# davidkelley/searchlite

Measured on NVIDIA B200. Metric: bm25_top10_queries_per_sec, higher is better.
Workload: dtype f32

## Files before the change

searchlite_b200/csrc/slg_host.h:

```cpp
#pragma once
#include "../../include/searchlite_gpu.h"

#include <algorithm>
#include <chrono>
#include <cmath>
#include <cstdarg>
#include <cstdio>
#include <cstdlib>
#include <cstring>
#include <limits>
#include <memory>
#include <string>
#include <unordered_map>
#include <vector>

#include <cuda_runtime.h>

#include "slg_launch.h"

namespace slg {

std::string &open_error();

cudaStream_t &pool_stream();
// ... 223 lines not shown
  slg_index *ix = nullptr;
  uint32_t Q = 0, k = 0, cap = 0, U = 0, T = 0;
  slg_exec_t exec = SLG_EXEC_BM25;
  bool matcher = false;
  bool want_stats = false;
  uint64_t posting_count = 0;
  slg::DevBuf slab;
  unsigned char *d_pack = nullptr;
  size_t pack_bytes = 0;
  size_t off_ut_term = 0, off_q_term_off = 0, off_qt_uterm = 0, off_qt_weight = 0, off_qt_group = 0, off_qt_flags = 0,
         off_q_order = 0, off_q_must = 0, off_q_not = 0, off_q_should = 0, off_q_min = 0, off_q_filter = 0,
         off_qt_leaf = 0, off_q_leaves = 0, off_q_plan_off = 0, off_plan_nodes = 0, off_cursor_bounds = 0;
  uint32_t *ut_rng = nullptr;
  float *ut_tile_ub = nullptr;
  unsigned char *state = nullptr;
  size_t state_bytes = 0;
  unsigned long long *thr_key = nullptr, *topk_keys = nullptr, *stats = nullptr, *item_counters = nullptr;
  uint32_t *topk_count = nullptr, *lock = nullptr, *work_counter = nullptr, *n_items = nullptr, *cursor_saw = nullptr;
  slg::QTerm *qterms = nullptr;
  slg::QHead *qheads = nullptr;
  uint2 *items = nullptr;
  slg::ColQ *colq = nullptr;
  uint32_t *ucol = nullptr, *col_slot = nullptr;
  float *ut_max = nullptr;
  slg::ScanPair *scan_pairs = nullptr;
  uint32_t *scan_order = nullptr, *scan_item_start = nullptr, *scan_items = nullptr;
  uint32_t scan_items_cap = 0, scan_chunk = 4096;
  uint32_t max_cols = 0;
  uint8_t *done = nullptr;
  size_t done_bytes = 0;
  uint32_t items_cap = 0;
  unsigned char *results = nullptr;
  size_t result_stride = 0;
  bool staged = false;
  uint32_t max_terms = 0;
  bool use_warp = false, can_items = false, canonical = false;
  bool and_scan = false;
  bool big_k = false;
  unsigned long long *pool_keys = nullptr;
  uint32_t *pool_count = nullptr, *pool_lock = nullptr;
  uint32_t pool_cap = 0;
  bool has_cursor = false;
  std::vector<uint8_t> h_has_cursor;
  uint32_t n_cursor_segs = 0;
  bool has_plan = false;
  uint32_t max_leaves = 1;
// ... 25 lines not shown
```

searchlite_b200/csrc/slg_launch.h:

```cpp
#pragma once
#include "slg_scan_kernel.cuh"

namespace slg {

cudaError_t launch_score_tiles(bool matcher, bool prune, bool stats, bool plan, const SegmentDev &sd, const BatchDev &bd, size_t smem,
                               int grid, cudaStream_t st);
cudaError_t launch_score_warp(bool matcher, bool prune, bool stats, bool staged, bool plan, const SegmentDev &sd, const WarpBatchDev &wb,
                              size_t smem, int grid, cudaStream_t st);
cudaError_t launch_score_items(bool prune, const SegmentDev &sd, const WarpBatchDev &wb, const ItemsDev &it, size_t smem, int grid,
                               cudaStream_t st);
cudaError_t launch_score_sparse(const SegmentDev &sd, const WarpBatchDev &wb, const StreamDev &st_dev, size_t smem, int grid, cudaStream_t st);
cudaError_t launch_score_columns(bool prune, bool pools, const SegmentDev &sd, const WarpBatchDev &wb, const StreamDev &st_dev, size_t smem, int grid, cudaStream_t st);
cudaError_t launch_scan(bool prune, bool pools, const SegmentDev &sd, const WarpBatchDev &wb, const ScanDev &sc, int grid, cudaStream_t st);
cudaError_t launch_columns_pruned(bool pools, const SegmentDev &sd, const WarpBatchDev &wb, const StreamDev &st_dev, int grid, cudaStream_t st);
cudaError_t launch_seed_items(const SegmentDev &sd, const WarpBatchDev &wb, const ItemsDev &it, size_t smem, int grid, cudaStream_t st);

}
```

searchlite_b200/csrc/slg_launch_items.cu:

```cuda
#include "slg_launch.h"

namespace slg {
namespace {
template <class K, class... A>
cudaError_t go(K kern, size_t smem, int grid, cudaStream_t st, A... args) {
  cudaError_t e = cudaFuncSetAttribute(kern, cudaFuncAttributeMaxDynamicSharedMemorySize, (int)smem);
  if (e != cudaSuccess) return e;
  kern<<<grid, kThreads, smem, st>>>(args...);
  return cudaGetLastError();
}
template <class K, class... A>
cudaError_t go_n(K kern, int threads, size_t smem, int grid, cudaStream_t st, A... args) {
  cudaError_t e = cudaFuncSetAttribute(kern, cudaFuncAttributeMaxDynamicSharedMemorySize, (int)smem);
  if (e != cudaSuccess) return e;
  kern<<<grid, threads, smem, st>>>(args...);
  return cudaGetLastError();
}
}

cudaError_t launch_score_items(bool prune, const SegmentDev &sd, const WarpBatchDev &wb, const ItemsDev &it, size_t smem, int grid,
                               cudaStream_t st) {
  return prune ? go(slg_score_items_kernel<true>, smem, grid, st, sd, wb, it) : go(slg_score_items_kernel<false>, smem, grid, st, sd, wb, it);
}
cudaError_t launch_score_sparse(const SegmentDev &sd, const WarpBatchDev &wb, const StreamDev &st_dev, size_t smem, int grid, cudaStream_t st) {
  cudaError_t e = cudaFuncSetAttribute(slg_score_sparse_kernel<false>, cudaFuncAttributeMaxDynamicSharedMemorySize, (int)smem);
  if (e != cudaSuccess) return e;
  slg_score_sparse_kernel<false><<<grid, kSparseWarps * 32, smem, st>>>(sd, wb, st_dev);
  return cudaGetLastError();
}
cudaError_t launch_score_columns(bool prune, bool pools, const SegmentDev &sd, const WarpBatchDev &wb, const StreamDev &st_dev, size_t smem, int grid,
                                 cudaStream_t st) {
  if (pools)
    return prune ? go_n(slg_score_columns_kernel<true, true>, kColWarps * 32, smem, grid, st, sd, wb, st_dev)
                 : go_n(slg_score_columns_kernel<false, true>, kColWarps * 32, smem, grid, st, sd, wb, st_dev);
  return prune ? go_n(slg_score_columns_kernel<true, false>, kColWarps * 32, smem, grid, st, sd, wb, st_dev)
               : go_n(slg_score_columns_kernel<false, false>, kColWarps * 32, smem, grid, st, sd, wb, st_dev);
}
cudaError_t launch_columns_pruned(bool pools, const SegmentDev &sd, const WarpBatchDev &wb, const StreamDev &st_dev, int grid, cudaStream_t st) {
  if (pools) slg_columns_pruned_kernel<1><<<grid, 256, 0, st>>>(sd, wb, st_dev);
  else slg_columns_pruned_kernel<0><<<grid, 256, 0, st>>>(sd, wb, st_dev);
  return cudaGetLastError();
}
template <bool PRUNE, bool POOLS>
static void launch_scan_pm(bool must, const SegmentDev &sd, const WarpBatchDev &wb, const ScanDev &sc, int grid, cudaStream_t st) {
  if (must) slg_scan_kernel<PRUNE, POOLS, true><<<grid, kScanWarps * 32, 0, st>>>(sd, wb, sc);
  else slg_scan_kernel<PRUNE, POOLS, false><<<grid, kScanWarps * 32, 0, st>>>(sd, wb, sc);
}
cudaError_t launch_scan(bool prune, bool pools, const SegmentDev &sd, const WarpBatchDev &wb, const ScanDev &sc, int grid, cudaStream_t st) {
  const bool must = sc.must_mode != 0u;
  if (pools) {
    if (prune) launch_scan_pm<true, true>(must, sd, wb, sc, grid, st);
    else launch_scan_pm<false, true>(must, sd, wb, sc, grid, st);
  } else {
    if (prune) launch_scan_pm<true, false>(must, sd, wb, sc, grid, st);
    else launch_scan_pm<false, false>(must, sd, wb, sc, grid, st);
  }
  return cudaGetLastError();
}
cudaError_t launch_seed_items(const SegmentDev &sd, const WarpBatchDev &wb, const ItemsDev &it, size_t smem, int grid, cudaStream_t st) {
  return go(slg_seed_items_kernel<0>, smem, grid, st, sd, wb, it);
}
}
```

searchlite_b200/csrc/slg_scan_kernel.cuh:

```cuda
#pragma once
#include "slg_stream_kernel.cuh"

namespace slg {

constexpr uint32_t kScanChunk = 4096;
constexpr int kScanWarps = 8;
constexpr uint32_t kScanQueue = 512;

struct __align__(16) ScanPair {
  uint64_t base;
  uint32_t df;
  uint32_t qslot_t;
  uint32_t qi;
  float w;
  float others;
  float ne_prefix;
  int32_t filter;
  uint32_t first_item;
  uint32_t pad[2];
};

struct ScanDev {
  const uint32_t *ut_term;
  float *ut_max;
// ... 22 lines not shown
  const uint32_t df = seg.term_df[term];
  const uint32_t quads = (df + 3) >> 2;
  const uint32_t per = (quads + gridDim.y - 1) / gridDim.y;
  const uint32_t q0 = blockIdx.y * per, q1 = min(quads, q0 + per);
  if (q0 >= q1) return;
  const float4 *p = reinterpret_cast<const float4 *>(seg.post_score + seg.term_start[term]);
  uint32_t m = 0u;
  for (uint32_t i = q0 + lane; i < q1; i += 32) {
    const float4 v = __ldg(p + i);
    m = max(m, max(max(__float_as_uint(v.x), __float_as_uint(v.y)), max(__float_as_uint(v.z), __float_as_uint(v.w))));
  }
  m = __reduce_max_sync(0xFFFFFFFFu, m);
  if (lane == 0 && m) atomicMax(reinterpret_cast<uint32_t *>(sc.ut_max) + u, m);
}

static __global__ void slg_term_ub_gather_kernel(SegmentDev seg, ScanDev sc, uint32_t n_uterms) {
  const uint32_t u = blockIdx.x * blockDim.x + threadIdx.x;
  if (u >= n_uterms) return;
  const uint32_t term = sc.ut_term[u];
  sc.ut_max[u] = term < seg.n_terms ? seg.term_ub[term] : 0.0f;
}

constexpr uint32_t kColSlices = 64;
template <int POOLS>
__global__ void __launch_bounds__(256) slg_columns_pruned_kernel(SegmentDev seg, WarpBatchDev wb, StreamDev sd) {
  __shared__ __align__(16) unsigned long long s_cand[8][kWarpCand];
  __shared__ uint32_t s_hist[8][POOLS ? 256 : 1];
  const int lane = threadIdx.x & 31, warp = threadIdx.x >> 5;
  const uint32_t n_colq = *sd.n_colq;
  const uint32_t wid = blockIdx.x * 8 + warp;
  const uint32_t qidx = wid / kColSlices, slice = wid % kColSlices;
  if (qidx >= n_colq) return;
  const ColQ cq = sd.colq[qidx];
  const QTerm *qts = wb.qterms + (uint64_t)cq.qslot * kWarpMaxTerms;
  const uint32_t nt = (uint32_t)cq.nsp + cq.ncol;
  const uint32_t n_blocks = (seg.doc_count + 511u) >> 9;
  const uint32_t per = (n_blocks + kColSlices - 1) / kColSlices;
  const uint32_t b0 = slice * per, b1 = min(n_blocks, b0 + per);
  WarpCand wc;
  wc.begin(s_cand[warp], load_threshold(wb, cq.qi), wb.k, lane, 1u, POOLS ? s_hist[warp] : nullptr);
  auto cut_of = [&]() {
    if (wc.thr == kThrInit) return 0u;
    const float cf = __uint_as_float((uint32_t)(wc.thr >> 32)) * 0.99998f - cq.extra * 1.00002f;
    return cf > 0.0f ? __float_as_uint(cf) : 0u;
  };
  for (uint32_t bb = b0; bb < b1; bb += 32) {
    const uint32_t blk = bb + lane;
    float bound = 0.0f;
    if (blk < b1)
      for (uint32_t i = 0; i < cq.ncol; i++) {
        const QTerm &q = qts[cq.nsp + i];
        bound = __fadd_rn(bound, __fmul_rn(__ldg(seg.col_tmax + (uint64_t)q.term * seg.tmax_stride + blk), q.weight));
      }
    uint32_t open = __ballot_sync(0xFFFFFFFFu, blk < b1 && bound != 0.0f && __float_as_uint(bound) >= cut_of());
    while (open) {
      const uint32_t d0 = (bb + (__ffs(open) - 1)) << 9;
      open &= open - 1;
      float4 v[4];
#pragma unroll
      for (int x = 0; x < 4; x++) v[x] = make_float4(0, 0, 0, 0);
      for (uint32_t i = 0; i < cq.ncol; i++) {
        const QTerm &q = qts[cq.nsp + i];
        const float4 *p = reinterpret_cast<const float4 *>(seg.cols + q.sc_base + d0) + lane;
        const float w = q.weight;
#pragma unroll
        for (int x = 0; x < 4; x++) {
          const float4 c = __ldg(p + x * 32);
          v[x].x = __fadd_rn(v[x].x, __fmul_rn(c.x, w));
          v[x].y = __fadd_rn(v[x].y, __fmul_rn(c.y, w));
          v[x].z = __fadd_rn(v[x].z, __fmul_rn(c.z, w));
          v[x].w = __fadd_rn(v[x].w, __fmul_rn(c.w, w));
        }
      }
      uint32_t cut = cut_of();
      uint32_t todo = 0u;
#pragma unroll
      for (int x = 0; x < 4; x++) {
        const uint32_t bx[4] = {__float_as_uint(v[x].x), __float_as_uint(v[x].y), __float_as_uint(v[x].z), __float_as_uint(v[x].w)};
#pragma unroll
        for (int e = 0; e < 4; e++)
          if (bx[e] >= cut && bx[e] != 0u && d0 + x * 128 + lane * 4 + e < seg.doc_count) todo |= 1u << (x * 4 + e);
      }
      while (__any_sync(0xFFFFFFFFu, todo != 0u)) {
        const uint32_t el = todo ? __ffs(todo) - 1 : 0u;
        const bool had = todo != 0u;
        todo &= todo - 1u;
        uint32_t bits = 0u;
#pragma unroll
        for (int x = 0; x < 4; x++) {
          if (el == (uint32_t)x * 4 + 0) bits = __float_as_uint(v[x].x);
          if (el == (uint32_t)x * 4 + 1) bits = __float_as_uint(v[x].y);
          if (el == (uint32_t)x * 4 + 2) bits = __float_as_uint(v[x].z);
          if (el == (uint32_t)x * 4 + 3) bits = __float_as_uint(v[x].w);
        }
        const uint32_t doc = d0 + (el >> 2) * 128 + lane * 4 + (el & 3u);
        cut = cut_of();
        const bool pass = had && bits >= cut;
        if (!__any_sync(0xFFFFFFFFu, pass)) continue;
        float s = __uint_as_float(bits);
        if (cq.nsp) {
          uint32_t holders = 0u;
          s = verify_doc(seg, wb, qts, nt, pass, doc, holders);
        }
        wc.offer(seg, wb, cq.qi, cq.filter, pass, doc, s);
      }
    }
  }
  wc.merge(wb, cq.qi);
}

static __global__ void __launch_bounds__(128) slg_scan_pairs_kernel(SegmentDev seg, WarpBatchDev wb, ScanDev sc, uint32_t dbg) {
  const uint32_t qslot = blockIdx.x * blockDim.x + threadIdx.x;
  if (qslot >= wb.n_queries) return;
  const QHead h = wb.qheads[qslot];
  float ub[kWarpMaxTerms];
  bool is_col[kWarpMaxTerms];
  for (uint32_t t = 0; t < kWarpMaxTerms; t++) {
    ub[t] = 0.0f;
    is_col[t] = false;
    if (t < h.nt) {
      const QTerm &q = wb.qterms[(uint64_t)qslot * kWarpMaxTerms + t];
      if (q.flags & 1u) ub[t] = __fmul_rn(sc.ut_max[q.uterm], q.weight);
      is_col[t] = (q.flags & 4u) != 0u;
    }
  }
  uint32_t driver = 0xFFFFFFFFu;
  float total_ub = 0.0f;
  if (sc.must_mode) {
    uint32_t best_df = 0xFFFFFFFFu;
    bool possible = h.nt > 0;
    for (uint32_t t = 0; t < h.nt && t < kWarpMaxTerms; t++) {
// ... 358 lines not shown
```

searchlite_b200/csrc/slg_search.cu:

```cuda
#include "slg_host.h"
#include "slg_residency.cuh"

using namespace slg;

namespace {

struct TermSet {
  std::vector<uint32_t> key, val;
  uint32_t mask = 0;
  explicit TermSet(size_t expect) {
    size_t n = 64;
    while (n < expect * 2) n <<= 1;
    key.assign(n, 0xFFFFFFFFu);
    val.assign(n, 0);
    mask = (uint32_t)n - 1;
  }
  uint32_t get(uint32_t term, std::vector<uint32_t> &ut) {
    uint32_t h = (term * 0x9E3779B1u) & mask;
    for (;;) {
      if (key[h] == term) return val[h];
      if (key[h] == 0xFFFFFFFFu) {
        key[h] = term;
        val[h] = (uint32_t)ut.size();
        ut.push_back(term);
        return val[h];
      }
// ... 245 lines not shown
    bt->off_q_leaves = place(n_queries);
    bt->off_q_plan_off = place((size_t)(n_queries + 1) * 4);
    bt->off_plan_nodes = place(plan_nodes.size() * sizeof(PlanNodeDev));
  }
  if (bt->has_cursor) bt->off_cursor_bounds = place(bounds.size() * 8);
  bt->pack_bytes = pos;

  size_t dpos = 0;
  auto carve = [&](size_t bytes) {
    size_t o = dpos;
    dpos = align_up(dpos + std::max<size_t>(bytes, 16), 256);
    return o;
  };
  const size_t o_pack = carve(bt->pack_bytes);
  const size_t o_rng = carve((size_t)std::max(bt->U, 1u) * (max_tiles + 1) * 4);
  const size_t o_ub = (exec != SLG_EXEC_BM25 || bt->can_items) ? carve((size_t)std::max(bt->U, 1u) * max_tiles * 4) : 0;
  uint32_t kp = 1;
  while (kp < k) kp <<= 1;
  bt->pool_cap = bt->big_k ? 2 * kp : 0;
  const size_t state_words = (size_t)n_queries * 2 + 64 + 2 + (bt->big_k ? (size_t)n_queries * 4 : 0);
  const size_t o_thr = carve((size_t)n_queries * 8 + state_words * 4);
  const size_t o_topk = carve((size_t)n_queries * k * 8);
  const size_t o_pools = bt->big_k ? carve((size_t)n_queries * 2 * bt->pool_cap * 8) : 0;
  const size_t o_stats = carve((size_t)n_queries * 5 * 8 + 64);
  const size_t o_saw = bt->has_cursor ? carve((size_t)n_queries * 4) : 0;
  const size_t o_qterms = bt->use_warp ? carve((size_t)n_queries * kWarpMaxTerms * sizeof(QTerm)) : 0;
  const size_t o_qheads = bt->use_warp ? carve((size_t)n_queries * sizeof(QHead)) : 0;
  const bool want_items = bt->can_items && exec != SLG_EXEC_BM25;
  bt->items_cap = want_items ? max_groups * n_queries : 0;
  bt->done_bytes = want_items ? (size_t)max_groups * n_queries : 0;
  const size_t o_items = want_items ? carve((size_t)bt->items_cap * sizeof(uint2)) : 0;
  const bool want_stream = bt->can_items && ix->stream_kernels;
  for (auto &s : ix->segs) bt->max_cols = std::max(bt->max_cols, s->n_cols);
  {
    uint32_t max_docs = 0;
    for (auto &sg : ix->segs) max_docs = std::max(max_docs, sg->doc_count);
    bt->scan_chunk = ix->scan_chunk ? ix->scan_chunk : (max_docs >= 4000000u ? 4096u : max_docs >= 2000000u ? 2048u : 1024u);
  }
  if (bt->can_items) {
    for (auto &sg : ix->segs) {
      uint64_t n = 0;
      for (size_t i = 0; i < qt_u.size(); i++) {
        const uint32_t term = ut[qt_u[i]];
        if (term >= sg->n_terms || !qt_f[i]) continue;
        if (!bt->and_scan && !sg->h_term_col.empty() && sg->h_term_col[term] >= 0) continue;
        n += (sg->h_df[term] + bt->scan_chunk - 1) / bt->scan_chunk;
      }
      bt->scan_items_cap = (uint32_t)std::max<uint64_t>(bt->scan_items_cap, std::min<uint64_t>(n, 0xFFFFFFF0ull));
    }
  }
  const bool want_scan = bt->can_items;
  const size_t o_utmax = want_scan ? carve((size_t)std::max(bt->U, 1u) * 4) : 0;
  const size_t o_pairs = want_scan ? carve((size_t)n_queries * kWarpMaxTerms * sizeof(ScanPair)) : 0;
  const size_t o_order = want_scan ? carve((size_t)n_queries * kWarpMaxTerms * 4) : 0;
  const size_t o_istart = want_scan ? carve(((size_t)n_queries * kWarpMaxTerms + 1) * 4) : 0;
  const size_t o_sitems = want_scan ? carve((size_t)std::max(bt->scan_items_cap, 1u) * 4) : 0;
  const size_t o_colq = want_stream ? carve((size_t)n_queries * sizeof(ColQ)) : 0;
  const size_t o_ucol = want_stream ? carve((size_t)(bt->max_cols + 1) * 4) : 0;
  const size_t o_colslot = want_stream ? carve((size_t)(bt->max_cols + 1) * 4) : 0;
  const size_t o_done = want_items ? carve(bt->done_bytes) : 0;
  bt->result_stride = align_up((size_t)n_queries * k * sizeof(HitDev) + (size_t)n_queries * 4 + (size_t)n_queries * k * 4, 256);
  const size_t o_results = carve(bt->result_stride * (S + (S > 1 ? 1 : 0)));
  SLG_CUDA(ix, bt->slab.alloc(dpos));
  unsigned char *base = bt->slab.as<unsigned char>();
  bt->d_pack = base + o_pack;
  bt->ut_rng = reinterpret_cast<uint32_t *>(base + o_rng);
  bt->ut_tile_ub = (exec != SLG_EXEC_BM25 || bt->can_items) ? reinterpret_cast<float *>(base + o_ub) : nullptr;
  bt->thr_key = reinterpret_cast<unsigned long long *>(base + o_thr);
  bt->state = base + o_thr + (size_t)n_queries * 8;
  bt->state_bytes = state_words * 4;
  bt->topk_count = reinterpret_cast<uint32_t *>(bt->state);
  bt->lock = bt->topk_count + n_queries;
  bt->work_counter = bt->lock + n_queries;
  bt->n_items = bt->work_counter + 64;
  bt->pool_count = bt->big_k ? bt->n_items + 2 : nullptr;
  bt->pool_lock = bt->big_k ? bt->pool_count + (size_t)n_queries * 2 : nullptr;
  bt->pool_keys = bt->big_k ? reinterpret_cast<unsigned long long *>(base + o_pools) : nullptr;
  bt->topk_keys = reinterpret_cast<unsigned long long *>(base + o_topk);
  bt->stats = reinterpret_cast<unsigned long long *>(base + o_stats);
  bt->item_counters = bt->stats + (size_t)n_queries * 5;
  bt->cursor_saw = bt->has_cursor ? reinterpret_cast<uint32_t *>(base + o_saw) : nullptr;
  bt->qterms = bt->use_warp ? reinterpret_cast<QTerm *>(base + o_qterms) : nullptr;
  bt->qheads = bt->use_warp ? reinterpret_cast<QHead *>(base + o_qheads) : nullptr;
  bt->items = want_items ? reinterpret_cast<uint2 *>(base + o_items) : nullptr;
  bt->done = want_items ? base + o_done : nullptr;
  bt->ut_max = want_scan ? reinterpret_cast<float *>(base + o_utmax) : nullptr;
  bt->scan_pairs = want_scan ? reinterpret_cast<ScanPair *>(base + o_pairs) : nullptr;
  bt->scan_order = want_scan ? reinterpret_cast<uint32_t *>(base + o_order) : nullptr;
  bt->scan_item_start = want_scan ? reinterpret_cast<uint32_t *>(base + o_istart) : nullptr;
  bt->scan_items = want_scan ? reinterpret_cast<uint32_t *>(base + o_sitems) : nullptr;
  bt->colq = want_stream ? reinterpret_cast<ColQ *>(base + o_colq) : nullptr;
  bt->ucol = want_stream ? reinterpret_cast<uint32_t *>(base + o_ucol) : nullptr;
  bt->col_slot = want_stream ? reinterpret_cast<uint32_t *>(base + o_colslot) : nullptr;
  bt->results = base + o_results;

  bt->pinned_result_off = align_up(bt->pack_bytes, 256);
  bt->pinned_bytes = bt->pinned_result_off + bt->result_stride + (size_t)n_queries * 40 + 64;
  if (!ix->pinned_busy && ix->pinned && ix->pinned_bytes >= bt->pinned_bytes) {
    bt->pinned = ix->pinned;
    bt->pinned_from_index = true;
    ix->pinned_busy = true;
  } else {
    SLG_CUDA(ix, cudaMallocHost(&bt->pinned, bt->pinned_bytes));
  }
  unsigned char *hp = static_cast<unsigned char *>(bt->pinned);
  auto put = [&](size_t off, const void *src, size_t bytes) {
    if (bytes) std::memcpy(hp + off, src, bytes);
  };
  put(bt->off_ut_term, ut.data(), (size_t)bt->U * 4);
  put(bt->off_q_term_off, q_off.data(), (size_t)(n_queries + 1) * 4);
  put(bt->off_qt_uterm, qt_u.data(), (size_t)bt->T * 4);
  put(bt->off_qt_weight, qt_w.data(), (size_t)bt->T * 4);
  put(bt->off_qt_group, qt_g.data(), bt->T);
  put(bt->off_qt_flags, qt_f.data(), bt->T);
  put(bt->off_q_order, order.data(), (size_t)n_queries * 4);
  put(bt->off_q_must, q_must.data(), n_queries);
  put(bt->off_q_not, q_not.data(), n_queries);
  put(bt->off_q_should, q_should.data(), n_queries);
  put(bt->off_q_min, q_min.data(), n_queries);
  put(bt->off_q_filter, q_filter.data(), (size_t)n_queries * 4);
// ... 20 lines not shown
  const bool prune = bt->exec != SLG_EXEC_BM25;
  const uint32_t Q = bt->Q, k = bt->k;
  const bool run_items = bt->can_items && !bt->want_stats && !(bt->big_k && (!ix->scan_kernels || (ix->strict_accumulate && bt->exec == SLG_EXEC_BM25)));
  const bool run_scan = run_items && ix->scan_kernels && bt->colq != nullptr && !(ix->strict_accumulate && !prune);
  if (bt->and_scan && !run_scan && run_items)
    return fail(ix, SLG_ERR_UNSUPPORTED, "an AND batch prepared for the posting scan cannot run on the sub-tile kernels (strict_accumulate)");
  const bool two_step = !(do_seeds && do_sweep);
  if (two_step && (ix->segs.size() != 1 || !run_items || (!prune && !run_scan)))
    return fail(ix, SLG_ERR_UNSUPPORTED, "the two-step run (first part, threshold exchange, rest) needs one segment per handle and the posting scan or the pruned items kernel");
  unsigned char *dp = bt->d_pack;
  size_t smem = 0;
  const bool run_scan_pre = bt->can_items && !bt->want_stats && ix->scan_kernels && bt->colq != nullptr && !(ix->strict_accumulate && !prune);
  const bool warp_path = bt->use_warp && !(bt->big_k && !run_scan_pre);
  if (!warp_path) {
    int32_t rc = bt->has_plan ? select_smem(ix, bt->plan_docs, bt->cap, bt->matcher, &smem, bt->max_leaves)
                              : select_smem(ix, ix->tile_docs, bt->cap, bt->matcher, &smem);
    if (rc) return rc;
  }
  uint32_t per_sm = (uint32_t)std::max<size_t>(1, (ix->smem_optin + 1024) / (smem + 1024));
  per_sm = std::min(per_sm, 8u);
  if (ix->ctas_per_sm) per_sm = std::min(per_sm, ix->ctas_per_sm);
  if (do_seeds) {
    SLG_CUDA(ix, cudaEventRecord(ix->ev[0], st));
    SLG_CUDA(ix, cudaMemsetAsync(bt->stats, 0, (size_t)Q * 40 + 64, st));
    if (bt->has_cursor) {
      if (bt->n_cursor_segs != ix->segs.size()) return fail(ix, SLG_ERR_INVALID, "a segment was loaded after the batch with cursors was prepared");
      SLG_CUDA(ix, cudaMemsetAsync(bt->cursor_saw, 0, (size_t)Q * 4, st));
    }
  }
  uint32_t si = 0;
  for (auto &sp : ix->segs) {
    Segment *s = sp.get();
    BatchDev bd{};
    bd.ut_term = reinterpret_cast<const uint32_t *>(dp + bt->off_ut_term);
    bd.ut_rng = bt->ut_rng;
    bd.ut_tile_ub = bt->ut_tile_ub;
    bd.q_term_off = reinterpret_cast<const uint32_t *>(dp + bt->off_q_term_off);
    bd.qt_uterm = reinterpret_cast<const uint32_t *>(dp + bt->off_qt_uterm);
    bd.qt_weight = reinterpret_cast<const float *>(dp + bt->off_qt_weight);
    bd.qt_group = dp + bt->off_qt_group;
    bd.qt_flags = dp + bt->off_qt_flags;
    bd.q_order = reinterpret_cast<const uint32_t *>(dp + bt->off_q_order);
    bd.q_must = dp + bt->off_q_must;
    bd.q_not = dp + bt->off_q_not;
    bd.q_should = dp + bt->off_q_should;
    bd.q_min_should = dp + bt->off_q_min;
    bd.q_filter = reinterpret_cast<const int32_t *>(dp + bt->off_q_filter);
// ... 127 lines not shown
      sc.ut_max = bt->ut_max;
      sc.pairs = bt->scan_pairs;
      sc.order = bt->scan_order;
      sc.n_pairs = bt->work_counter + 5;
      sc.n_items = bt->work_counter + 6;
      sc.item_start = bt->scan_item_start;
      sc.items = bt->scan_items;
      sc.items_cap = bt->scan_items_cap;
      sc.chunk = bt->scan_chunk;
      sc.must_mode = bt->and_scan ? 1u : 0u;
      sc.counter = bt->work_counter + 7;
      sc.counters = bt->item_counters;
      StreamDev sdv{};
      sdv.colq = bt->colq;
      sdv.n_colq = bt->work_counter + 3;
      sdv.ucol = bt->ucol;
      sdv.n_ucol = bt->work_counter + 4;
      sdv.col_slot = bt->col_slot;
      sdv.sparse_counter = bt->work_counter + 1;
      sdv.col_counter = bt->work_counter + 2;
      sdv.stage_cap = ix->stage_cap;
      sdv.strict = 0;
      sdv.counters = bt->item_counters;
      if (do_seeds) {
        if (prune && s->dev.term_ub) {
          slg_term_ub_gather_kernel<<<(bt->U + 255) / 256, 256, 0, st>>>(s->dev, sc, bt->U);
        } else {
          SLG_CUDA(ix, cudaMemsetAsync(bt->ut_max, 0, (size_t)bt->U * 4, st));
          slg_term_max_kernel<<<dim3((bt->U + 7) / 8, kMaxSlices), 256, 0, st>>>(s->dev, sc, bt->U);
        }
        slg_scan_pairs_kernel<<<(Q + 127) / 128, 128, 0, st>>>(s->dev, wb, sc, ix->dbg);
        slg_scan_order_kernel<<<1, 1024, 0, st>>>(wb, sc);
        if (bt->scan_items_cap) slg_scan_items_kernel<<<(bt->scan_items_cap + 255) / 256, 256, 0, st>>>(sc);
        for (int i = 0; i < 4; i++) count_launch(ix);
        SLG_CUDA(ix, cudaGetLastError());
        SLG_CUDA(ix, cudaEventRecord(ix->ev[2], st));
      }
      sc.two_rounds = (ix->dbg & 8u) ? 1u : 0u;
      sc.part_lo = do_seeds ? 0u : ix->scan_first_part;
      sc.part_hi = do_sweep ? 256u : ix->scan_first_part;
      SLG_CUDA(ix, launch_scan(prune, wb.pool_keys != nullptr, s->dev, wb, sc, ix->n_sm * 4, st));
      count_launch(ix);
      if (do_sweep && s->n_cols && !(ix->dbg & 4u) && !bt->and_scan) {
        slg_colgroups_kernel<<<1, 1024, 0, st>>>(s->dev, wb, sdv, s->n_cols, prune ? bt->ut_max : nullptr);
        count_launch(ix);
        SLG_CUDA(ix, cudaGetLastError());
        sdv.n_smax = std::min(s->n_cols, kColMaxSlots);
        const size_t fixed = column_smem(0, sdv.n_smax);
        const size_t reserve = 2048 + (size_t)kColWarps * 256 * 4;
        const size_t budget = ix->smem_optin > fixed + reserve ? ix->smem_optin - fixed - reserve : 0;
        sdv.col_resident = (uint32_t)std::min<size_t>(s->n_cols, budget / (2 * kColBlock * 4));
        const size_t csmem = column_smem(sdv.col_resident, sdv.n_smax);
        const uint32_t n_cblocks = (s->doc_count + kColBlock - 1) / kColBlock;
        if (prune) {
          (void)csmem;
          (void)n_cblocks;
          SLG_CUDA(ix, launch_columns_pruned(wb.pool_keys != nullptr, s->dev, wb, sdv, (int)((Q * kColSlices + 7) / 8), st));
        } else {
          SLG_CUDA(ix, launch_score_columns(false, wb.pool_keys != nullptr, s->dev, wb, sdv, csmem, (int)std::min<uint32_t>((uint32_t)ix->n_sm, n_cblocks), st));
        }
        count_launch(ix);
      }
      if (do_sweep) ix->ctr.score_launches++;
    }
    if (do_sweep) {
      if (score && run_scan) {
      } else if (score && run_stream) {
        StreamDev sdv{};
        sdv.colq = bt->colq;
        sdv.n_colq = bt->work_counter + 3;
        sdv.ucol = bt->ucol;
        sdv.n_ucol = bt->work_counter + 4;
        sdv.col_slot = bt->col_slot;
        sdv.sparse_counter = bt->work_counter + 1;
        sdv.col_counter = bt->work_counter + 2;
        sdv.stage_cap = ix->stage_cap;
        sdv.strict = ix->strict_accumulate;
        sdv.counters = bt->item_counters;
        const size_t ssmem = (size_t)kSparseWarps * sparse_smem_per_warp(wb.sub_docs, sdv.stage_cap);
        if (ssmem + 1024 > ix->smem_optin) return fail(ix, SLG_ERR_UNSUPPORTED, "sub_docs %u with stage_cap %u needs %zu B shared memory", wb.sub_docs, sdv.stage_cap, ssmem);
// ... 177 lines not shown
}

int32_t slg_batch_device_results(slg_batch_t *bt, void **dev_hits, void **dev_counts) {
  if (!bt || !dev_hits || !dev_counts) return SLG_ERR_INVALID;
  unsigned char *r = result_block(bt);
  *dev_hits = r;
  *dev_counts = r + (size_t)bt->Q * bt->k * sizeof(HitDev);
  return SLG_OK;
}

int32_t slg_batch_packed_results(slg_batch_t *bt, void **dev_block, uint64_t *n_bytes) {
  if (!bt || !dev_block || !n_bytes) return SLG_ERR_INVALID;
  *dev_block = result_block(bt);
  *n_bytes = (uint64_t)bt->Q * bt->k * sizeof(HitDev) + (uint64_t)bt->Q * 4 + (bt->reranked ? (uint64_t)bt->Q * bt->k * 4 : 0);
  return SLG_OK;
}

int32_t slg_batch_fetch(slg_batch_t *bt, slg_hit_t *out_hits, uint32_t *out_counts, slg_stats_t *out_stats) {
  if (!bt || !out_hits || !out_counts) return SLG_ERR_INVALID;
  slg_index *ix = bt->ix;
  SLG_CUDA(ix, cudaSetDevice(ix->device));
  cudaStream_t st = ix->stream;
  static_assert(sizeof(slg_hit_t) == sizeof(HitDev), "hit layout");
  const size_t hb = (size_t)bt->Q * bt->k * sizeof(slg_hit_t), cb = (size_t)bt->Q * 4, sb = (size_t)bt->Q * 40 + 64;
  unsigned char *pin = static_cast<unsigned char *>(bt->pinned) + bt->pinned_result_off;
  SLG_CUDA(ix, cudaMemcpyAsync(pin, result_block(bt), hb + cb, cudaMemcpyDeviceToHost, st));
  SLG_CUDA(ix, cudaMemcpyAsync(pin + bt->result_stride, bt->stats, sb, cudaMemcpyDeviceToHost, st));
  SLG_CUDA(ix, cudaStreamSynchronize(st));
  ix->ctr.last_d2h_bytes = hb + cb + sb;
  std::memcpy(out_hits, pin, hb);
  std::memcpy(out_counts, pin + hb, cb);
  const unsigned long long *sv = reinterpret_cast<const unsigned long long *>(pin + bt->result_stride);
  const unsigned long long *ic = sv + (size_t)bt->Q * 5;
  ix->ctr.last_postings_scattered = ic[0];
  ix->ctr.last_subtiles_skipped = ic[1];
  ix->ctr.last_column_blocks_streamed = ic[2];
  ix->ctr.last_items = ic[3];
  ix->ctr.last_postings_verified = ic[4];
  ix->ctr.last_items_dropped = ic[5];
  if (getenv("SLG_SCAN_TRACE"))
    fprintf(stderr, "[slg scan] verified %llu, sparse look-ups answered by a presence bitmap %llu, by lower_bound_interp %llu\n", ic[4], ic[6], ic[7]);
  if (out_stats) {
    for (uint32_t q = 0; q < bt->Q; q++) {
      out_stats[q].scored_docs = sv[q * 4 + 0];
      out_stats[q].postings_advanced = sv[q * 4 + 1];
      out_stats[q].blocks_skipped = sv[q * 4 + 2];
      out_stats[q].candidates_examined = sv[q * 4 + 3];
      out_stats[q].total_matches = sv[(size_t)bt->Q * 4 + q];
    }
  }
  return SLG_OK;
}

int32_t slg_batch_copy_results_device(slg_batch_t *bt, void *dst_hits, void *dst_counts) {
  if (!bt || !dst_hits || !dst_counts) return SLG_ERR_INVALID;
  slg_index *ix = bt->ix;
  SLG_CUDA(ix, cudaSetDevice(ix->device));
  void *dh, *dc;
  slg_batch_device_results(bt, &dh, &dc);
  SLG_CUDA(ix, cudaMemcpyAsync(dst_hits, dh, (size_t)bt->Q * bt->k * sizeof(HitDev), cudaMemcpyDeviceToDevice, ix->stream));
  SLG_CUDA(ix, cudaMemcpyAsync(dst_counts, dc, (size_t)bt->Q * 4, cudaMemcpyDeviceToDevice, ix->stream));
  return SLG_OK;
}

// ... 115 lines not shown
```

searchlite_b200/csrc/slg_stream_kernel.cuh:

```cuda
#pragma once
#include "slg_async.cuh"
#include "slg_items_kernel.cuh"
#include "slg_residency.cuh"

namespace slg {

constexpr uint32_t kColBlock = 256;
constexpr int kSparseWarps = 4;
constexpr int kColWarps = 16;
constexpr uint32_t kColMaxSlots = 4096;

struct __align__(16) ColQ {
  uint32_t qslot, qi;
  int32_t filter;
  uint8_t nsp, ncol, unit_w, off;
  uint16_t slot[8];
  float extra;
  uint32_t pad[3];
};

struct StreamDev {
  ColQ *colq;
  uint32_t *n_colq;
  uint32_t *ucol;
  uint32_t *n_ucol;
  uint32_t *col_slot;
  uint32_t *sparse_counter, *col_counter;
  uint32_t stage_cap;
  uint32_t col_resident;
  uint32_t n_smax;
  uint32_t strict;
  unsigned long long *counters;
};

__device__ __forceinline__ bool colq_prune(const WarpBatchDev &wb, const float *ut_max, uint32_t qslot, uint32_t qi, uint32_t nt, float &extra) {
  const unsigned long long thr = load_threshold(wb, qi);
  float ub[kWarpMaxTerms];
  bool col[kWarpMaxTerms];
  for (uint32_t t = 0; t < kWarpMaxTerms; t++) {
    ub[t] = 0.0f;
    col[t] = false;
    if (t < nt) {
      const QTerm &q = wb.qterms[(uint64_t)qslot * kWarpMaxTerms + t];
      if (q.flags & 1u) ub[t] = __fmul_rn(ut_max[q.uterm], q.weight);
      col[t] = (q.flags & 5u) == 5u;
    }
  }
  extra = 0.0f;
  bool any_essential_col = false;
  for (uint32_t t = 0; t < nt; t++) {
    float pre = 0.0f;
    for (uint32_t u = 0; u < nt; u++)
      if (ub[u] < ub[t] || (ub[u] == ub[t] && u >= t)) pre += ub[u];
    const bool ne = thr != kThrInit && pre * 1.00002f < __uint_as_float((uint32_t)(thr >> 32));
    if (col[t]) any_essential_col = any_essential_col || !ne;
// ... 45 lines not shown
          sd.col_slot[c] = 0xFFFFFFFFu;
        }
      }
      __syncthreads();
      if (tid == nthr - 1) s_carry += s_scan[tid];
      __syncthreads();
    }
    if (tid == 0) *sd.n_ucol = s_carry;
  }
  __syncthreads();
  for (uint32_t slot = tid; slot < wb.n_queries; slot += nthr) {
    const QHead h = wb.qheads[slot];
    ColQ r;
    r.qslot = slot;
    r.qi = h.qi;
    r.filter = h.filter;
    r.nsp = 0;
    r.ncol = 0;
    r.unit_w = 1;
    r.off = 0;
    r.extra = 0.0f;
    r.pad[0] = r.pad[1] = r.pad[2] = 0;
    for (int i = 0; i < 8; i++) r.slot[i] = 0;
    for (uint32_t t = 0; t < h.nt; t++) {
      const QTerm &q = wb.qterms[(uint64_t)slot * kWarpMaxTerms + t];
      if (!(q.flags & 1u)) continue;
      if (q.flags & 4u) {
        r.slot[r.ncol++] = (uint16_t)sd.col_slot[q.term];
        if (q.weight != 1.0f) r.unit_w = 0;
      } else {
        r.nsp++;
      }
    }
    if (r.ncol && ut_max) {
      if (!colq_prune(wb, ut_max, slot, h.qi, h.nt, r.extra)) continue;
      bool all_in = true;
      for (uint32_t i = 0; i < r.ncol; i++) all_in = all_in && r.slot[i] != 0xFFFFu;
      if (!all_in) r.off = 1;
    }
    if (r.ncol && !r.off) sd.colq[atomicAdd(sd.n_colq, 1u)] = r;
  }
}

__device__ __forceinline__ uint32_t warp_dedupe64(unsigned long long *a, int lane) {
  const unsigned long long x0 = a[lane], x1 = a[lane + 32];
  const unsigned long long p0 = lane ? a[lane - 1] : ~0ull, p1 = a[lane + 31];
  const bool k0 = x0 != 0ull && x0 != p0, k1 = x1 != 0ull && x1 != p1;
  const uint32_t b0 = __ballot_sync(0xFFFFFFFFu, k0), b1 = __ballot_sync(0xFFFFFFFFu, k1);
  const uint32_t lt = (1u << lane) - 1u, n0 = __popc(b0), n = n0 + __popc(b1);
  __syncwarp();
  if (k0) a[__popc(b0 & lt)] = x0;
  if (k1) a[n0 + __popc(b1 & lt)] = x1;
  __syncwarp();
  for (uint32_t z = n + lane; z < kWarpCand; z += 32) a[z] = 0ull;
  __syncwarp();
  return n;
}

struct WarpCand {
  unsigned long long *cand;
  unsigned long long thr;
  uint32_t cnt;
  uint32_t k;
// ... 78 lines not shown
    if (k1 <= thr) k1 = 0ull;
    const uint32_t b0 = __ballot_sync(0xFFFFFFFFu, k0 != 0ull), b1 = __ballot_sync(0xFFFFFFFFu, k1 != 0ull);
    const uint32_t n_new = __popc(b0) + __popc(b1);
    cnt = 0;
    __syncwarp();
    if (n_new == 0) return;
    const uint32_t slot = qi * 2u + pool;
    unsigned long long *pk = wb.pool_keys + (uint64_t)slot * wb.pool_cap;
    if (lane == 0) {
      while (atomicCAS(wb.pool_lock + slot, 0u, 1u) != 0u) __nanosleep(64);
      __threadfence();
    }
    __syncwarp();
    uint32_t n = ld_cg_u32(wb.pool_count + slot);
    if (n + n_new > wb.pool_cap) n = compact_pool(wb, qi, pk, n);
    const uint32_t lt = (1u << lane) - 1u;
    const uint32_t w0 = __ballot_sync(0xFFFFFFFFu, k0 > thr), w1 = __ballot_sync(0xFFFFFFFFu, k1 > thr);
    if (k0 > thr) st_cg_u64(pk + n + __popc(w0 & lt), k0);
    if (k1 > thr) st_cg_u64(pk + n + __popc(w0) + __popc(w1 & lt), k1);
    __threadfence();
    __syncwarp();
    if (lane == 0) {
      st_cg_u32(wb.pool_count + slot, n + __popc(w0) + __popc(w1));
      __threadfence();
      atomicExch(wb.pool_lock + slot, 0u);
    }
    __syncwarp();
  }
  __device__ __forceinline__ void push(bool pass, unsigned long long key) {
    const uint32_t bal = __ballot_sync(0xFFFFFFFFu, pass);
    if (!bal) return;
    if (pass) cand[cnt + __popc(bal & ((1u << lane) - 1u))] = key;
    cnt += __popc(bal);
    __syncwarp();
    if (cnt > 32 && hist) {
      return;
    }
    if (cnt > 32) {
      for (uint32_t z = cnt + lane; z < kWarpCand; z += 32) cand[z] = 0ull;
      __syncwarp();
      warp_sort64_desc(cand, lane);
      cnt = min(warp_dedupe64(cand, lane), k);
      if (cnt == k) thr = max(thr, cand[k - 1]);
      __syncwarp();
    }
  }
// ... 775 lines not shown
```

Before: 593,100.

## Seed column-pruned scoring with best-bound blocks per query to raise thresholds early

```diff
diff --git a/searchlite_b200/csrc/slg_host.h b/searchlite_b200/csrc/slg_host.h
--- a/searchlite_b200/csrc/slg_host.h
+++ b/searchlite_b200/csrc/slg_host.h
@@ -269,6 +269,7 @@
   uint2 *items = nullptr;
   slg::ColQ *colq = nullptr;
   uint32_t *ucol = nullptr, *col_slot = nullptr;
+  uint32_t *col_seeded = nullptr;
   float *ut_max = nullptr;
   slg::ScanPair *scan_pairs = nullptr;
   uint32_t *scan_order = nullptr, *scan_item_start = nullptr, *scan_items = nullptr;
diff --git a/searchlite_b200/csrc/slg_launch.h b/searchlite_b200/csrc/slg_launch.h
--- a/searchlite_b200/csrc/slg_launch.h
+++ b/searchlite_b200/csrc/slg_launch.h
@@ -12,7 +12,7 @@
 cudaError_t launch_score_sparse(const SegmentDev &sd, const WarpBatchDev &wb, const StreamDev &st_dev, size_t smem, int grid, cudaStream_t st);
 cudaError_t launch_score_columns(bool prune, bool pools, const SegmentDev &sd, const WarpBatchDev &wb, const StreamDev &st_dev, size_t smem, int grid, cudaStream_t st);
 cudaError_t launch_scan(bool prune, bool pools, const SegmentDev &sd, const WarpBatchDev &wb, const ScanDev &sc, int grid, cudaStream_t st);
-cudaError_t launch_columns_pruned(bool pools, const SegmentDev &sd, const WarpBatchDev &wb, const StreamDev &st_dev, int grid, cudaStream_t st);
+cudaError_t launch_columns_pruned(bool pools, const SegmentDev &sd, const WarpBatchDev &wb, const StreamDev &st_dev, uint32_t n_queries, cudaStream_t st);
 cudaError_t launch_seed_items(const SegmentDev &sd, const WarpBatchDev &wb, const ItemsDev &it, size_t smem, int grid, cudaStream_t st);
 
 }
diff --git a/searchlite_b200/csrc/slg_launch_items.cu b/searchlite_b200/csrc/slg_launch_items.cu
--- a/searchlite_b200/csrc/slg_launch_items.cu
+++ b/searchlite_b200/csrc/slg_launch_items.cu
@@ -36,9 +36,15 @@
   return prune ? go_n(slg_score_columns_kernel<true, false>, kColWarps * 32, smem, grid, st, sd, wb, st_dev)
                : go_n(slg_score_columns_kernel<false, false>, kColWarps * 32, smem, grid, st, sd, wb, st_dev);
 }
-cudaError_t launch_columns_pruned(bool pools, const SegmentDev &sd, const WarpBatchDev &wb, const StreamDev &st_dev, int grid, cudaStream_t st) {
-  if (pools) slg_columns_pruned_kernel<1><<<grid, 256, 0, st>>>(sd, wb, st_dev);
-  else slg_columns_pruned_kernel<0><<<grid, 256, 0, st>>>(sd, wb, st_dev);
+cudaError_t launch_columns_pruned(bool pools, const SegmentDev &sd, const WarpBatchDev &wb, const StreamDev &st_dev, uint32_t n_queries, cudaStream_t st) {
+  const int grid = (int)(((uint64_t)n_queries * kColSlices + 7) / 8);
+  if (pools) {
+    slg_columns_seed_kernel<1><<<n_queries, kColSeeds, 0, st>>>(sd, wb, st_dev);
+    slg_columns_pruned_kernel<1><<<grid, 256, 0, st>>>(sd, wb, st_dev);
+  } else {
+    slg_columns_seed_kernel<0><<<n_queries, kColSeeds, 0, st>>>(sd, wb, st_dev);
+    slg_columns_pruned_kernel<0><<<grid, 256, 0, st>>>(sd, wb, st_dev);
+  }
   return cudaGetLastError();
 }
 template <bool PRUNE, bool POOLS>
diff --git a/searchlite_b200/csrc/slg_scan_kernel.cuh b/searchlite_b200/csrc/slg_scan_kernel.cuh
--- a/searchlite_b200/csrc/slg_scan_kernel.cuh
+++ b/searchlite_b200/csrc/slg_scan_kernel.cuh
@@ -68,6 +68,126 @@
 }
 
 constexpr uint32_t kColSlices = 64;
+#ifndef SLG_COL_SEED_WARPS
+#define SLG_COL_SEED_WARPS 8
+#endif
+constexpr uint32_t kColSeedWarps = SLG_COL_SEED_WARPS;
+constexpr uint32_t kColSeeds = kColSeedWarps * 32;
+constexpr int kSeedBatch = 8;
+
+__device__ __forceinline__ uint32_t col_cut(unsigned long long thr, float extra) {
+  if (thr == kThrInit) return 0u;
+  const float cf = __uint_as_float((uint32_t)(thr >> 32)) * 0.99998f - extra * 1.00002f;
+  return cf > 0.0f ? __float_as_uint(cf) : 0u;
+}
+
+__device__ __forceinline__ void col_score_block(const SegmentDev &seg, const WarpBatchDev &wb, const ColQ &cq, const QTerm *qts, uint32_t d0,
+                                                WarpCand &wc, int lane) {
+  const uint32_t nt = (uint32_t)cq.nsp + cq.ncol;
+  float4 v[4];
+#pragma unroll
+  for (int x = 0; x < 4; x++) v[x] = make_float4(0, 0, 0, 0);
+  for (uint32_t i = 0; i < cq.ncol; i++) {
+    const QTerm &q = qts[cq.nsp + i];
+    const float4 *p = reinterpret_cast<const float4 *>(seg.cols + q.sc_base + d0) + lane;
+    const float w = q.weight;
+#pragma unroll
+    for (int x = 0; x < 4; x++) {
+      const float4 c = __ldg(p + x * 32);
+      v[x].x = __fadd_rn(v[x].x, __fmul_rn(c.x, w));
+      v[x].y = __fadd_rn(v[x].y, __fmul_rn(c.y, w));
+      v[x].z = __fadd_rn(v[x].z, __fmul_rn(c.z, w));
+      v[x].w = __fadd_rn(v[x].w, __fmul_rn(c.w, w));
+    }
+  }
+  uint32_t cut = col_cut(wc.thr, cq.extra);
+  uint32_t todo = 0u;
+#pragma unroll
+  for (int x = 0; x < 4; x++) {
+    const uint32_t bx[4] = {__float_as_uint(v[x].x), __float_as_uint(v[x].y), __float_as_uint(v[x].z), __float_as_uint(v[x].w)};
+#pragma unroll
+    for (int e = 0; e < 4; e++)
+      if (bx[e] >= cut && bx[e] != 0u && d0 + x * 128 + lane * 4 + e < seg.doc_count) todo |= 1u << (x * 4 + e);
+  }
+  while (__any_sync(0xFFFFFFFFu, todo != 0u)) {
+    const uint32_t el = todo ? __ffs(todo) - 1 : 0u;
+    const bool had = todo != 0u;
+    todo &= todo - 1u;
+    uint32_t bits = 0u;
+#pragma unroll
+    for (int x = 0; x < 4; x++) {
+      if (el == (uint32_t)x * 4 + 0) bits = __float_as_uint(v[x].x);
+      if (el == (uint32_t)x * 4 + 1) bits = __float_as_uint(v[x].y);
+      if (el == (uint32_t)x * 4 + 2) bits = __float_as_uint(v[x].z);
+      if (el == (uint32_t)x * 4 + 3) bits = __float_as_uint(v[x].w);
+    }
+    const uint32_t doc = d0 + (el >> 2) * 128 + lane * 4 + (el & 3u);
+    cut = col_cut(wc.thr, cq.extra);
+    const bool pass = had && bits >= cut;
+    if (!__any_sync(0xFFFFFFFFu, pass)) continue;
+    float s = __uint_as_float(bits);
+    if (cq.nsp) {
+      uint32_t holders = 0u;
+      s = verify_doc(seg, wb, qts, nt, pass, doc, holders);
+    }
+    wc.offer(seg, wb, cq.qi, cq.filter, pass, doc, s);
+  }
+}
+
+template <int POOLS>
+__global__ void __launch_bounds__(kColSeedWarps * 32, 1) slg_columns_seed_kernel(SegmentDev seg, WarpBatchDev wb, StreamDev sd) {
+  __shared__ __align__(16) unsigned long long s_cand[kColSeedWarps][kWarpCand];
+  __shared__ uint32_t s_hist[kColSeedWarps][POOLS ? 256 : 1];
+  const int lane = threadIdx.x & 31, warp = threadIdx.x >> 5;
+  const uint32_t qidx = blockIdx.x, g = threadIdx.x;
+  if (qidx >= *sd.n_colq) return;
+  const ColQ cq = sd.colq[qidx];
+  const QTerm *qts = wb.qterms + (uint64_t)cq.qslot * kWarpMaxTerms;
+  const uint32_t n_blocks = (seg.doc_count + 511u) >> 9;
+  float best = 0.0f;
+  uint32_t best_blk = 0xFFFFFFFFu;
+  for (uint32_t b0 = g; b0 < n_blocks; b0 += kColSeeds * kSeedBatch) {
+    float bnd[kSeedBatch];
+#pragma unroll
+    for (int j = 0; j < kSeedBatch; j++) bnd[j] = 0.0f;
+    for (uint32_t i = 0; i < cq.ncol; i++) {
+      const QTerm &q = qts[cq.nsp + i];
+      const float *tm = seg.col_tmax + (uint64_t)q.term * seg.tmax_stride;
+      const float w = q.weight;
+#pragma unroll
+      for (int j = 0; j < kSeedBatch; j++) {
+        const uint32_t blk = b0 + j * kColSeeds;
+        if (blk < n_blocks) bnd[j] = __fadd_rn(bnd[j], __fmul_rn(__ldg(tm + blk), w));
+      }
+    }
+#pragma unroll
+    for (int j = 0; j < kSeedBatch; j++)
+      if (bnd[j] > best) {
+        best = bnd[j];
+        best_blk = b0 + j * kColSeeds;
+      }
+  }
+  sd.seeded[(uint64_t)qidx * kColSeeds + g] = best_blk;
+  WarpCand wc;
+  wc.begin(s_cand[warp], load_threshold(wb, cq.qi), wb.k, lane, 1u, POOLS ? s_hist[warp] : nullptr);
+  bool left = best_blk != 0xFFFFFFFFu;
+  uint32_t n_open = 0;
+  for (;;) {
+    wc.thr = max(wc.thr, load_threshold(wb, cq.qi));
+    const uint32_t bits = left ? __float_as_uint(best) : 0u;
+    const uint32_t top = __reduce_max_sync(0xFFFFFFFFu, bits);
+    if (top == 0u || top < col_cut(wc.thr, cq.extra)) break;
+    const uint32_t owner = __ffs(__ballot_sync(0xFFFFFFFFu, left && bits == top)) - 1;
+    if (lane == (int)owner) left = false;
+    const uint32_t blk = __shfl_sync(0xFFFFFFFFu, best_blk, owner);
+    n_open++;
+    col_score_block(seg, wb, cq, qts, blk << 9, wc, lane);
+  }
+  if (POOLS) wc.publish_pool(wb, cq.qi);
+  else wc.merge(wb, cq.qi);
+  if (sd.counters && lane == 0 && n_open) atomicAdd(sd.counters + 1, (unsigned long long)n_open);
+}
+
 template <int POOLS>
 __global__ void __launch_bounds__(256) slg_columns_pruned_kernel(SegmentDev seg, WarpBatchDev wb, StreamDev sd) {
   __shared__ __align__(16) unsigned long long s_cand[8][kWarpCand];
@@ -79,18 +199,17 @@
   if (qidx >= n_colq) return;
   const ColQ cq = sd.colq[qidx];
   const QTerm *qts = wb.qterms + (uint64_t)cq.qslot * kWarpMaxTerms;
-  const uint32_t nt = (uint32_t)cq.nsp + cq.ncol;
   const uint32_t n_blocks = (seg.doc_count + 511u) >> 9;
   const uint32_t per = (n_blocks + kColSlices - 1) / kColSlices;
   const uint32_t b0 = slice * per, b1 = min(n_blocks, b0 + per);
+  const uint32_t *seeded = sd.seeded + (uint64_t)qidx * kColSeeds;
   WarpCand wc;
   wc.begin(s_cand[warp], load_threshold(wb, cq.qi), wb.k, lane, 1u, POOLS ? s_hist[warp] : nullptr);
-  auto cut_of = [&]() {
-    if (wc.thr == kThrInit) return 0u;
-    const float cf = __uint_as_float((uint32_t)(wc.thr >> 32)) * 0.99998f - cq.extra * 1.00002f;
-    return cf > 0.0f ? __float_as_uint(cf) : 0u;
-  };
-  for (uint32_t bb = b0; bb < b1; bb += 32) {
+  for (uint32_t bb = b0;; bb += 32) {
+    const unsigned long long thr_now = load_threshold(wb, cq.qi);
+    if (bb >= b1 || (!POOLS && wc.thr > thr_now)) wc.merge(wb, cq.qi);
+    if (bb >= b1) break;
+    wc.thr = max(wc.thr, thr_now);
     const uint32_t blk = bb + lane;
     float bound = 0.0f;
     if (blk < b1)
@@ -98,61 +217,16 @@
         const QTerm &q = qts[cq.nsp + i];
         bound = __fadd_rn(bound, __fmul_rn(__ldg(seg.col_tmax + (uint64_t)q.term * seg.tmax_stride + blk), q.weight));
       }
-    uint32_t open = __ballot_sync(0xFFFFFFFFu, blk < b1 && bound != 0.0f && __float_as_uint(bound) >= cut_of());
+    const bool seeded_here = blk < b1 && __ldg(seeded + blk % kColSeeds) == blk;
+    uint32_t open = __ballot_sync(0xFFFFFFFFu, blk < b1 && !seeded_here && bound != 0.0f && __float_as_uint(bound) >= col_cut(wc.thr, cq.extra));
+    if (sd.counters && lane == 0 && open) atomicAdd(sd.counters + 1, (unsigned long long)__popc(open));
     while (open) {
       const uint32_t d0 = (bb + (__ffs(open) - 1)) << 9;
       open &= open - 1;
-      float4 v[4];
-#pragma unroll
-      for (int x = 0; x < 4; x++) v[x] = make_float4(0, 0, 0, 0);
-      for (uint32_t i = 0; i < cq.ncol; i++) {
-        const QTerm &q = qts[cq.nsp + i];
-        const float4 *p = reinterpret_cast<const float4 *>(seg.cols + q.sc_base + d0) + lane;
-        const float w = q.weight;
-#pragma unroll
-        for (int x = 0; x < 4; x++) {
-          const float4 c = __ldg(p + x * 32);
-          v[x].x = __fadd_rn(v[x].x, __fmul_rn(c.x, w));
-          v[x].y = __fadd_rn(v[x].y, __fmul_rn(c.y, w));
-          v[x].z = __fadd_rn(v[x].z, __fmul_rn(c.z, w));
-          v[x].w = __fadd_rn(v[x].w, __fmul_rn(c.w, w));
-        }
-      }
-      uint32_t cut = cut_of();
-      uint32_t todo = 0u;
-#pragma unroll
-      for (int x = 0; x < 4; x++) {
-        const uint32_t bx[4] = {__float_as_uint(v[x].x), __float_as_uint(v[x].y), __float_as_uint(v[x].z), __float_as_uint(v[x].w)};
-#pragma unroll
-        for (int e = 0; e < 4; e++)
-          if (bx[e] >= cut && bx[e] != 0u && d0 + x * 128 + lane * 4 + e < seg.doc_count) todo |= 1u << (x * 4 + e);
-      }
-      while (__any_sync(0xFFFFFFFFu, todo != 0u)) {
-        const uint32_t el = todo ? __ffs(todo) - 1 : 0u;
-        const bool had = todo != 0u;
-        todo &= todo - 1u;
-        uint32_t bits = 0u;
-#pragma unroll
-        for (int x = 0; x < 4; x++) {
-          if (el == (uint32_t)x * 4 + 0) bits = __float_as_uint(v[x].x);
-          if (el == (uint32_t)x * 4 + 1) bits = __float_as_uint(v[x].y);
-          if (el == (uint32_t)x * 4 + 2) bits = __float_as_uint(v[x].z);
-          if (el == (uint32_t)x * 4 + 3) bits = __float_as_uint(v[x].w);
-        }
-        const uint32_t doc = d0 + (el >> 2) * 128 + lane * 4 + (el & 3u);
-        cut = cut_of();
-        const bool pass = had && bits >= cut;
-        if (!__any_sync(0xFFFFFFFFu, pass)) continue;
-        float s = __uint_as_float(bits);
-        if (cq.nsp) {
-          uint32_t holders = 0u;
-          s = verify_doc(seg, wb, qts, nt, pass, doc, holders);
-        }
-        wc.offer(seg, wb, cq.qi, cq.filter, pass, doc, s);
-      }
-    }
-  }
-  wc.merge(wb, cq.qi);
+      col_score_block(seg, wb, cq, qts, d0, wc, lane);
+    }
+  }
+  if (sd.counters && lane == 0 && b0 < b1) atomicAdd(sd.counters + 2, (unsigned long long)(b1 - b0));
 }
 
 static __global__ void __launch_bounds__(128) slg_scan_pairs_kernel(SegmentDev seg, WarpBatchDev wb, ScanDev sc, uint32_t dbg) {
diff --git a/searchlite_b200/csrc/slg_search.cu b/searchlite_b200/csrc/slg_search.cu
--- a/searchlite_b200/csrc/slg_search.cu
+++ b/searchlite_b200/csrc/slg_search.cu
@@ -2,6 +2,8 @@
 #include "slg_residency.cuh"
 
 using namespace slg;
+
+constexpr size_t kItemCounterBytes = 10 * 8;
 
 namespace {
 
@@ -293,7 +295,7 @@
   const size_t o_thr = carve((size_t)n_queries * 8 + state_words * 4);
   const size_t o_topk = carve((size_t)n_queries * k * 8);
   const size_t o_pools = bt->big_k ? carve((size_t)n_queries * 2 * bt->pool_cap * 8) : 0;
-  const size_t o_stats = carve((size_t)n_queries * 5 * 8 + 64);
+  const size_t o_stats = carve((size_t)n_queries * 5 * 8 + kItemCounterBytes);
   const size_t o_saw = bt->has_cursor ? carve((size_t)n_queries * 4) : 0;
   const size_t o_qterms = bt->use_warp ? carve((size_t)n_queries * kWarpMaxTerms * sizeof(QTerm)) : 0;
   const size_t o_qheads = bt->use_warp ? carve((size_t)n_queries * sizeof(QHead)) : 0;
@@ -327,6 +329,7 @@
   const size_t o_istart = want_scan ? carve(((size_t)n_queries * kWarpMaxTerms + 1) * 4) : 0;
   const size_t o_sitems = want_scan ? carve((size_t)std::max(bt->scan_items_cap, 1u) * 4) : 0;
   const size_t o_colq = want_stream ? carve((size_t)n_queries * sizeof(ColQ)) : 0;
+  const size_t o_seeded = want_stream ? carve((size_t)n_queries * kColSeeds * 4) : 0;
   const size_t o_ucol = want_stream ? carve((size_t)(bt->max_cols + 1) * 4) : 0;
   const size_t o_colslot = want_stream ? carve((size_t)(bt->max_cols + 1) * 4) : 0;
   const size_t o_done = want_items ? carve(bt->done_bytes) : 0;
@@ -361,12 +364,13 @@
   bt->scan_item_start = want_scan ? reinterpret_cast<uint32_t *>(base + o_istart) : nullptr;
   bt->scan_items = want_scan ? reinterpret_cast<uint32_t *>(base + o_sitems) : nullptr;
   bt->colq = want_stream ? reinterpret_cast<ColQ *>(base + o_colq) : nullptr;
+  bt->col_seeded = want_stream ? reinterpret_cast<uint32_t *>(base + o_seeded) : nullptr;
   bt->ucol = want_stream ? reinterpret_cast<uint32_t *>(base + o_ucol) : nullptr;
   bt->col_slot = want_stream ? reinterpret_cast<uint32_t *>(base + o_colslot) : nullptr;
   bt->results = base + o_results;
 
   bt->pinned_result_off = align_up(bt->pack_bytes, 256);
-  bt->pinned_bytes = bt->pinned_result_off + bt->result_stride + (size_t)n_queries * 40 + 64;
+  bt->pinned_bytes = bt->pinned_result_off + bt->result_stride + (size_t)n_queries * 40 + kItemCounterBytes;
   if (!ix->pinned_busy && ix->pinned && ix->pinned_bytes >= bt->pinned_bytes) {
     bt->pinned = ix->pinned;
     bt->pinned_from_index = true;
@@ -433,7 +437,7 @@
   if (ix->ctas_per_sm) per_sm = std::min(per_sm, ix->ctas_per_sm);
   if (do_seeds) {
     SLG_CUDA(ix, cudaEventRecord(ix->ev[0], st));
-    SLG_CUDA(ix, cudaMemsetAsync(bt->stats, 0, (size_t)Q * 40 + 64, st));
+    SLG_CUDA(ix, cudaMemsetAsync(bt->stats, 0, (size_t)Q * 40 + kItemCounterBytes, st));
     if (bt->has_cursor) {
       if (bt->n_cursor_segs != ix->segs.size()) return fail(ix, SLG_ERR_INVALID, "a segment was loaded after the batch with cursors was prepared");
       SLG_CUDA(ix, cudaMemsetAsync(bt->cursor_saw, 0, (size_t)Q * 4, st));
@@ -607,6 +611,7 @@
       sdv.stage_cap = ix->stage_cap;
       sdv.strict = 0;
       sdv.counters = bt->item_counters;
+      sdv.seeded = bt->col_seeded;
       if (do_seeds) {
         if (prune && s->dev.term_ub) {
           slg_term_ub_gather_kernel<<<(bt->U + 255) / 256, 256, 0, st>>>(s->dev, sc, bt->U);
@@ -640,7 +645,8 @@
         if (prune) {
           (void)csmem;
           (void)n_cblocks;
-          SLG_CUDA(ix, launch_columns_pruned(wb.pool_keys != nullptr, s->dev, wb, sdv, (int)((Q * kColSlices + 7) / 8), st));
+          SLG_CUDA(ix, launch_columns_pruned(wb.pool_keys != nullptr, s->dev, wb, sdv, Q, st));
+          count_launch(ix);
         } else {
           SLG_CUDA(ix, launch_score_columns(false, wb.pool_keys != nullptr, s->dev, wb, sdv, csmem, (int)std::min<uint32_t>((uint32_t)ix->n_sm, n_cblocks), st));
         }
@@ -864,7 +870,7 @@
   SLG_CUDA(ix, cudaSetDevice(ix->device));
   cudaStream_t st = ix->stream;
   static_assert(sizeof(slg_hit_t) == sizeof(HitDev), "hit layout");
-  const size_t hb = (size_t)bt->Q * bt->k * sizeof(slg_hit_t), cb = (size_t)bt->Q * 4, sb = (size_t)bt->Q * 40 + 64;
+  const size_t hb = (size_t)bt->Q * bt->k * sizeof(slg_hit_t), cb = (size_t)bt->Q * 4, sb = (size_t)bt->Q * 40 + kItemCounterBytes;
   unsigned char *pin = static_cast<unsigned char *>(bt->pinned) + bt->pinned_result_off;
   SLG_CUDA(ix, cudaMemcpyAsync(pin, result_block(bt), hb + cb, cudaMemcpyDeviceToHost, st));
   SLG_CUDA(ix, cudaMemcpyAsync(pin + bt->result_stride, bt->stats, sb, cudaMemcpyDeviceToHost, st));
@@ -881,7 +887,10 @@
   ix->ctr.last_postings_verified = ic[4];
   ix->ctr.last_items_dropped = ic[5];
   if (getenv("SLG_SCAN_TRACE"))
-    fprintf(stderr, "[slg scan] verified %llu, sparse look-ups answered by a presence bitmap %llu, by lower_bound_interp %llu\n", ic[4], ic[6], ic[7]);
+    fprintf(stderr,
+            "[slg scan] verified %llu, sparse look-ups answered by a presence bitmap %llu, by lower_bound_interp %llu; "
+            "column pass: %llu queries with a scanned sparse term, %llu without\n",
+            ic[4], ic[6], ic[7], ic[8], ic[9]);
   if (out_stats) {
     for (uint32_t q = 0; q < bt->Q; q++) {
       out_stats[q].scored_docs = sv[q * 4 + 0];
diff --git a/searchlite_b200/csrc/slg_stream_kernel.cuh b/searchlite_b200/csrc/slg_stream_kernel.cuh
--- a/searchlite_b200/csrc/slg_stream_kernel.cuh
+++ b/searchlite_b200/csrc/slg_stream_kernel.cuh
@@ -31,6 +31,7 @@
   uint32_t n_smax;
   uint32_t strict;
   unsigned long long *counters;
+  uint32_t *seeded;
 };
 
 __device__ __forceinline__ bool colq_prune(const WarpBatchDev &wb, const float *ut_max, uint32_t qslot, uint32_t qi, uint32_t nt, float &extra) {
@@ -122,6 +123,7 @@
     r.extra = 0.0f;
     r.pad[0] = r.pad[1] = r.pad[2] = 0;
     for (int i = 0; i < 8; i++) r.slot[i] = 0;
+    bool scanned = false;
     for (uint32_t t = 0; t < h.nt; t++) {
       const QTerm &q = wb.qterms[(uint64_t)slot * kWarpMaxTerms + t];
       if (!(q.flags & 1u)) continue;
@@ -130,6 +132,7 @@
         if (q.weight != 1.0f) r.unit_w = 0;
       } else {
         r.nsp++;
+        scanned = scanned || q.term < seg.n_terms;
       }
     }
     if (r.ncol && ut_max) {
@@ -138,7 +141,10 @@
       for (uint32_t i = 0; i < r.ncol; i++) all_in = all_in && r.slot[i] != 0xFFFFu;
       if (!all_in) r.off = 1;
     }
-    if (r.ncol && !r.off) sd.colq[atomicAdd(sd.n_colq, 1u)] = r;
+    if (r.ncol && !r.off) {
+      sd.colq[atomicAdd(sd.n_colq, 1u)] = r;
+      if (sd.counters) atomicAdd(sd.counters + (scanned ? 8 : 9), 1ull);
+    }
   }
 }
 
@@ -263,6 +269,27 @@
     __syncwarp();
     if (lane == 0) {
       st_cg_u32(wb.pool_count + slot, n + __popc(w0) + __popc(w1));
+      __threadfence();
+      atomicExch(wb.pool_lock + slot, 0u);
+    }
+    __syncwarp();
+  }
+  __device__ __forceinline__ void publish_pool(const WarpBatchDev &wb, uint32_t qi) {
+    flush(wb, qi);
+    const uint32_t slot = qi * 2u + pool;
+    if (lane == 0) {
+      while (atomicCAS(wb.pool_lock + slot, 0u, 1u) != 0u) __nanosleep(64);
+      __threadfence();
+    }
+    __syncwarp();
+    const uint32_t n = ld_cg_u32(wb.pool_count + slot);
+    if (n >= k) {
+      const uint32_t kept = compact_pool(wb, qi, wb.pool_keys + (uint64_t)slot * wb.pool_cap, n);
+      __threadfence();
+      __syncwarp();
+      if (lane == 0) st_cg_u32(wb.pool_count + slot, kept);
+    }
+    if (lane == 0) {
       __threadfence();
       atomicExch(wb.pool_lock + slot, 0u);
     }
```

Result: faster. 626,700, median of 6 (+5.7%).
